# mkangquantum/quits

Hardware: AMD Instinct MI355X
Metric: decoded shots/sec + logical-error-rate, [[144,12,12]] BB code, d rounds, p=0.003 (higher is better)
Workload: dtype f32

## Files before the change

quits_amd/csrc/bp_scatter_wide.hip:

```cpp
#include "qd_internal.h"
#include "qd_host.h"
#include "../../include/quits_amd.h"
#include "bp_scatter_edge.h"

#define QSW_GATHER_PRIO(j_) if ((j_) == 0) __builtin_amdgcn_s_setprio(0); else if ((j_) == CPL - 1) __builtin_amdgcn_s_setprio(2); else __builtin_amdgcn_s_setprio(1);

template <int T, int MW, int CPL, int NSW>
__global__ void __launch_bounds__(T, MW) qd_bp_scatter_wide_kernel(BpGraphDev g, ScatGraphDev sg, DecodeArgs a, ScatArgs x)
{
    extern __shared__ __align__(16) unsigned char smem[];
    const uint32_t lds_base = (uint32_t)(uintptr_t)(__attribute__((address_space(3))) unsigned char *)smem;
    if (lds_base != 0u) __builtin_trap();
    uint32_t *outw = reinterpret_cast<uint32_t *>(smem + sg.off_out);
    int *misc = reinterpret_cast<int *>(smem + sg.off_misc);
    constexpr int NW = T / 64;
    static_assert(T % 64 == 0 && NW <= 16, "workgroup shape");

    const int tid = threadIdx.x;
    const int64_t shot = blockIdx.x;
    const uint8_t *det = a.det + shot * a.det_stride + a.det_offset;
    const uint8_t *upd = a.upd ? a.upd + shot * a.upd_stride : nullptr;
    const int m_pad = g.m_pad, n_pad = g.n_pad;

    int any = 0;
// ... 284 lines not shown
            }
            return;
        }
    }
    for (int b = tid; b < sg.nslots; b += T)
        if (*QS_LDS(cur + 4u * (uint32_t)b) < 0) {
            const uint32_t jf = sg.slot_fault[b];
            if (jf != 0xFFFFFFFFu) atomicOr(&outw[jf >> 5], 1u << (jf & 31u));
        }
    if (!converged && a.want_llr && tid == 0) misc[48] = atomicAdd(a.fail_count, 1);
    __syncthreads();
    for (int w = tid; w < g.out_words; w += T) a.err_bits[shot * g.out_words + w] = outw[w];
    if (!converged && a.want_llr) {
        const int slot = misc[48];
        float *dst = a.llr_ws + (int64_t)slot * n_pad;
        for (int k1 = tid; k1 < g.n; k1 += T) dst[k1] = (float)(*QS_LDS(cur + 4u * sg.k1_slot[k1]) + 1) * x.grid_inv;
        if (tid == 0) a.fail_list[slot] = (int32_t)shot;
    }
    if (tid == 0) a.status[shot] = t | (converged * QD_STATUS_CONVERGED) | a.status_or;
}

#undef QS_ACC
#define QS_ACC(off) (prior_g[((uint32_t)(off) - (uint32_t)sg.offA) >> 2])
#define QS_ADJ(row_) qs_as_uint4(__builtin_amdgcn_raw_buffer_load_b128(adj_rsrc, adj_voff, (row_) * adj_row, 0))
template <int NSW>
__global__ void __launch_bounds__(64) qd_bp_first_pass_kernel(BpGraphDev g, ScatGraphDev sg, const int32_t *prior_g, uint32_t *rec)
{
    static_assert(NSW == 3, "the record has room for three sign words");
    const int c = (int)blockIdx.x * 64 + (int)threadIdx.x;
    const bool actv = c < g.m;
    constexpr int j = 0;
// ... 66 lines not shown
```

quits_amd/csrc/graph_layout.h:

```cpp
#pragma once
#include "qd_graph_views.h"

#include <cstddef>
#include <memory>
#include <type_traits>
#include <utility>
#include <vector>

#define QD_GEN_PREFIX_LDS (32 * 1024)

int qd_fail(int code, const char *fmt, ...);

struct Switches {
    bool no_scatter, scatter_cpl1, scatter_wide_t704, scatter_natural_rounds, scatter_banks_by_slot, scatter_walk_greedy, osdcs_old, bp_no_fast_start;
    float scatter_m2_limit;
    std::vector<int> gen_stages;
};
Switches qd_read_switches();

struct HostGraph {
    int m = 0, n = 0, nnz = 0, max_rdeg = 0, max_cdeg = 0, min_rdeg = 0, m_pad = 0, n_pad = 0, max_rdeg_pad = 0;
    const int32_t *row_ptr = nullptr, *col_idx = nullptr;
    const double *priors = nullptr;
    std::vector<int> rdeg, cdeg;
    std::vector<double> llr0;
    std::vector<int32_t> cp, ri, pos;
    std::vector<int> chk_orig, chk_slot_of, bit_orig, bit_slot_of;
    std::vector<uint8_t> chk_deg;
};
int qd_host_graph(int32_t m, int32_t n, const int32_t *row_ptr, const int32_t *col_idx, const double *priors, HostGraph &h);
// ... 39 lines not shown
```

quits_amd/csrc/graph_layout.hip:

```cpp
#include "graph_layout.h"
#include "../../include/quits_amd.h"

#include <algorithm>
#include <cmath>
#include <cstdlib>
#include <cstring>
#include <numeric>


static inline int align16(int x) { return (x + 15) & ~15; }
static inline int pad64(int x) { return (x + 63) & ~63; }

Switches qd_read_switches()
{
    auto env = [](const char *name) { return std::getenv(name); };
    Switches w{};
    w.no_scatter = env("QD_NO_SCATTER") != nullptr;
    w.scatter_cpl1 = env("QD_SCATTER_CPL1") != nullptr;
    w.scatter_wide_t704 = env("QD_SCATTER_WIDE_T704") != nullptr;
    w.scatter_natural_rounds = env("QD_SCATTER_NATURAL_ROUNDS") != nullptr;
    w.scatter_banks_by_slot = env("QD_SCATTER_BANKS_BY_SLOT") != nullptr;
    w.scatter_walk_greedy = env("QD_SCATTER_WALK_GREEDY") != nullptr;
    const char *ev = env("QD_BP_NO_FAST_START");
    w.bp_no_fast_start = ev && std::atoi(ev) == 1;
    ev = env("QD_OSDCS_OLD");
    w.osdcs_old = ev && std::atoi(ev) == 1;
    ev = env("QD_SCATTER_M2_LIMIT");
    w.scatter_m2_limit = ev ? (float)std::atof(ev) : INFINITY;
    w.gen_stages = {3, 6, 10, 14, 20, 28, 40, 56, 80, 112};
    if ((ev = env("QD_GEN_STAGES"))) {
        w.gen_stages.clear();
        for (const char *q = ev; *q;) {
            char *end = nullptr;
            const long v = std::strtol(q, &end, 10);
            if (end == q) break;
            if (v > 0) w.gen_stages.push_back((int)v);
            q = *end ? end + 1 : end;
        }
    }
    return w;
}

static void scatter_banks(int m, int n, const int32_t *row_ptr, const int32_t *col_idx, const std::vector<int> &chk_orig,
// ... 647 lines not shown
```

quits_amd/csrc/osd_shared.h:

```cpp
#pragma once
#include "qd_internal.h"

#define QD_NOKEY 0xFFFFFFFFu

#ifdef QD_OSD_TIMING
#define QD_TICK(slot)                                                                   \
    {                                                                                   \
        const unsigned long long now_ = wall_clock64();                                 \
        acc_[slot] += now_ - tick_;                                                     \
        tick_ = now_;                                                                   \
    }
#else
#define QD_TICK(slot)
#endif

__device__ __forceinline__ uint64_t &qd_qword(uint64_t *q_lds, uint64_t *q_glb, int kw_lds, int m_pad, int w, int r)
{
    return (w < kw_lds) ? q_lds[(size_t)w * m_pad + r] : q_glb[(size_t)(w - kw_lds) * m_pad + r];
}

__device__ __forceinline__ uint32_t qd_mono_key(float llr)
{
    const float f = llr + 0.0f;
    const uint32_t u = __float_as_uint(f);
    return (u & 0x80000000u) ? ~u : (u | 0x80000000u);
}

template <int T>
__device__ __forceinline__ void qd_bitonic_u64(uint64_t *buf, int P, int tid)
{
    for (int k = 2; k <= P; k <<= 1)
        for (int j = k >> 1; j > 0; j >>= 1) {
            for (int pi = tid; pi < (P >> 1); pi += T) {
                const int i = ((pi & ~(j - 1)) << 1) | (pi & (j - 1));
                const int l = i | j;
                const uint64_t x = buf[i], y = buf[l];
                const bool up = ((i & k) == 0);
                if ((x > y) == up) { buf[i] = y; buf[l] = x; }
            }
            __syncthreads();
// ... 34 lines not shown
    const uint8_t *det, *upd;
    int64_t det_stride, det_offset, upd_stride;
    const float *llr_ws;
    const int32_t *fail_list, *fail_count;
    const int32_t *slot_list, *slot_count;
    uint64_t *q_spill_fast;
    uint64_t *mt_ws;
    uint32_t *err_bits;
    int32_t *status;
    unsigned long long *dbg;
};

struct TierState {
    uint32_t lo_key, lo_idx; int sphase, exhausted, limit;
    uint32_t guess = 0u, cut = 0u, count = 0u;
};

template <int T, int KPT = QD_OSD_KPT, class ARGS = OsdRegArgs, int SCAN = 0>
__device__ __forceinline__ int qd_osd_draw_tier(const ARGS &a, const float *llr, uint64_t *sortbuf, uint16_t *order,
                                             uint32_t *red, uint32_t *sumbuf, TierState &ts)
{
    const int tid = threadIdx.x;
    const int n = a.n;
    const bool in_regs = n <= KPT * T;
    uint32_t lo_key = ts.lo_key, lo_idx = ts.lo_idx;
    int sphase = ts.sphase;
    const uint32_t lim = (uint32_t)ts.limit;
    bool exhausted = false;
    int cnt = 0;
    {
            uint32_t kreg[KPT];
            if (in_regs) {
#pragma unroll
                for (int i = 0; i < KPT; ++i) {
                    const int b = tid + i * T;
                    kreg[i] = (b < n) ? qd_mono_key(llr[b]) : 0xFFFFFFFFu;
                }
            }
            auto scan_keys = [&](auto fn) {
                if constexpr (SCAN == 0) {
                    for (int b = tid; b < n; b += T) fn(qd_mono_key(llr[b]), b);
                } else {
                    const float4 *l4 = reinterpret_cast<const float4 *>(llr);
                    const int n4 = n >> 2;
                    for (int b0 = 0; b0 < n4; b0 += SCAN * T) {
                        float4 v[SCAN > 0 ? SCAN : 1];
#pragma unroll
                        for (int u = 0; u < SCAN; ++u) {
                            const int b4 = b0 + u * T + tid;
                            v[u] = l4[b4 < n4 ? b4 : 0];
                        }
#pragma unroll
                        for (int u = 0; u < SCAN; ++u) {
                            const int b4 = b0 + u * T + tid;
// ... 7 lines not shown
                }
            };
            auto count_ties = [&](uint32_t key, uint32_t ilo, uint32_t ihi) -> uint32_t {
                uint32_t c = 0;
                for (int b = tid; b < n; b += T)
                    if (qd_mono_key(llr[b]) == key) { const uint32_t j = a.bit_orig[b]; c += (j >= ilo && j < ihi) ? 1u : 0u; }
                return qd_block_sum<T>(c, sumbuf, sphase);
            };
            bool by_index = false;
            uint32_t t_lo = lo_key, t_hi = lo_key, i_lo = 0, i_hi = 0;
            if (lo_idx > 0) {
                if (count_ties(lo_key, lo_idx, 0xFFFFFFFFu) > 0) by_index = true;
                else { lo_key += 1; lo_idx = 0; }
            }
            bool spec = !by_index && !in_regs && ts.guess > lo_key;
            for (;;) {
            if (spec) { t_lo = lo_key; t_hi = (uint32_t)__builtin_amdgcn_readfirstlane((int)ts.guess); }
            else {
            if (!by_index) {
                uint32_t *hist = reinterpret_cast<uint32_t *>(sortbuf);
                uint32_t base = 0u, cur_lo = lo_key, cum = 0u;
                uint64_t thi64 = 0;
                for (int level = 0; level < 3; ++level) {
                    const int shift = level == 0 ? 21 : (level == 1 ? 10 : 0);
                    const int nb = level == 2 ? 1024 : 2048;
                    for (int i = tid; i < nb; i += T) hist[i] = 0u;
                    __syncthreads();
                    auto tally = [&](uint32_t u) {
                        if (u != 0xFFFFFFFFu && u >= cur_lo) {
                            const uint32_t bin = (u - base) >> shift;
                            if (bin < (uint32_t)nb) atomicAdd(&hist[bin], 1u);
                        }
// ... 84 lines not shown
            scan_keys([&](uint32_t u, int b) {
                bool take = false;
                uint32_t j = 0;
                if (by_index) { if (u == t_lo) { j = a.bit_orig[b]; take = (j >= i_lo && j < i_hi); } }
                else if (u >= t_lo && u < t_hi) { j = a.bit_orig[b]; take = true; }
                if (take) {
                    const uint32_t at = atomicAdd(&red[80], 1u);
                    if (at < (uint32_t)QD_OSD_TIER) sortbuf[at] = ((uint64_t)u << 32) | j;
                }
            });
            __syncthreads();
            if (!spec) break;
            {
                const uint32_t c = (uint32_t)__builtin_amdgcn_readfirstlane((int)red[80]);
                ts.count = c;
                if (c > 0u && c <= lim) { cnt = (int)c; lo_key = t_hi; ts.cut = t_hi; break; }
                spec = false;
                __syncthreads();
            }
            }
            int P = 64;
            while (P < cnt) P <<= 1;
            for (int i = cnt + tid; i < P; i += T) sortbuf[i] = ~0ull;
            __syncthreads();
            if (cnt <= 256 && cnt <= T) {
                if ((tid & ~63) < cnt) {
                    const uint64_t mine = tid < cnt ? sortbuf[tid] : ~0ull;
                    const uint4 *sb4 = reinterpret_cast<const uint4 *>(sortbuf);
                    int rank = 0;
                    for (int i = 0; i < (cnt + 1) / 2; ++i) {
                        const uint4 v = sb4[i];
                        const uint64_t k0 = (uint64_t)v.x | ((uint64_t)v.y << 32), k1 = (uint64_t)v.z | ((uint64_t)v.w << 32);
                        rank += (k0 < mine ? 1 : 0) + (k1 < mine ? 1 : 0);
                    }
                    if (tid < cnt) order[rank] = (uint16_t)(mine & 0xFFFFu);
                }
            } else {
                qd_bitonic_u64<T>(sortbuf, P, tid);
                for (int i = tid; i < cnt; i += T) order[i] = (uint16_t)(sortbuf[i] & 0xFFFFu);
            }
            __syncthreads();
    }
    ts.lo_key = lo_key; ts.lo_idx = lo_idx; ts.sphase = sphase; ts.exhausted = 0;
    return cnt;
}

struct OsdLds {
    uint64_t *q;
    uint64_t *tb;
    uint8_t *sp;
    int16_t *rowpiv;
    uint16_t *prow;
    uint32_t *pcol;
    uint32_t *pairs;
    uint32_t *bcols;
    uint32_t *red;
    uint32_t *outw;
};
// ... 176 lines not shown
```

quits_amd/csrc/osd_sr.hip:

```cpp
#include "osd_shared.h"
#include "qd_host.h"
#include <algorithm>

#define QD_SR_KWR 4
struct OsdSrArgs {
    int m, n, m_pad, n_pad, mw, out_words, upd_rows, ell_log2;
    int o_tb, o_rowpiv, o_prow, o_pcol, o_ppos, o_nz, o_cand, o_stq, o_stsp, o_bcols, o_red, o_out, o_order;
    int tier_first;
    const uint16_t *csc_ell;
    const uint32_t *bit_orig;
    const uint8_t *det, *upd;
    int64_t det_stride, det_offset, upd_stride;
    const float *llr_ws;
    const int32_t *fail_list, *fail_count;
    uint64_t *q_spill;
    int32_t *hard_list, *hard_count;
    uint32_t *err_bits;
    int32_t *status;
    unsigned long long *dbg;
};

template <int T, int RPT, int KWR>
__global__ void __launch_bounds__(T, qd_sr_wps(RPT)) qd_osd0_sr_kernel(OsdSrArgs a)
{
    extern __shared__ __align__(16) unsigned char smem[];
    const int tid = threadIdx.x, lane = tid & 63;
    constexpr int NW = T / 64;
    static_assert(NW <= 16 && T >= 256, "key / flag records hold 16 wavefronts; the tier drawing wants >= 256 threads");
    uint64_t *tb = reinterpret_cast<uint64_t *>(smem + a.o_tb);
// ... 2 lines not shown
    uint16_t *prow = reinterpret_cast<uint16_t *>(smem + a.o_prow);
    uint32_t *pcol = reinterpret_cast<uint32_t *>(smem + a.o_pcol);
    uint16_t *ppos = reinterpret_cast<uint16_t *>(smem + a.o_ppos);
    uint64_t *nz = reinterpret_cast<uint64_t *>(smem + a.o_nz);
    uint32_t *cand = reinterpret_cast<uint32_t *>(smem + a.o_cand);
    uint64_t *stq = reinterpret_cast<uint64_t *>(smem + a.o_stq);
    uint32_t *stsp = reinterpret_cast<uint32_t *>(smem + a.o_stsp);
    uint32_t *bcols = reinterpret_cast<uint32_t *>(smem + a.o_bcols);
    uint32_t *red = reinterpret_cast<uint32_t *>(smem + a.o_red);
    uint32_t *sumbuf = red + 96;
    uint32_t *outw = reinterpret_cast<uint32_t *>(smem + a.o_out);
    uint16_t *order = reinterpret_cast<uint16_t *>(smem + a.o_order);
    const int m = a.m, m_pad = a.m_pad, mw = a.mw, dlog = a.ell_log2;
    uint64_t *qglb = a.q_spill + (size_t)blockIdx.x * (size_t)(mw > KWR ? mw - KWR : 0) * m_pad;
    const int nfail = *a.fail_count;
    if (tid == 0) red[81] = 0u;
    for (int item = blockIdx.x; item < nfail; item += gridDim.x) {
        const int slot = item;
        const int64_t shot = a.fail_list[slot];
        const float *llr = a.llr_ws + (int64_t)slot * a.n_pad;
        const uint8_t *det = a.det + shot * a.det_stride + a.det_offset;
        const uint8_t *upd = a.upd ? a.upd + shot * a.upd_stride : nullptr;
#ifdef QD_OSD_TIMING
        unsigned long long acc_[12] = {0, 0, 0, 0, 0, 0, 0, 0, 0, 0, 0, 0};
        unsigned long long tick_ = wall_clock64();
#endif
        uint64_t my_tb[RPT], my_q[RPT][KWR];
        uint32_t my_sp = 0, my_piv = 0;
#pragma unroll
        for (int i = 0; i < RPT; ++i) {
// ... 11 lines not shown
        }
        for (int w = tid; w < a.out_words; w += T) outw[w] = 0u;
        if (tid < 240) cand[tid] = (tid % 80) < 64 ? QD_NOKEY : 0u;
        if (tid == 0) red[72] = 0u;
        __syncthreads();
        QD_TICK(10)

        int npiv = 0, done = 0, draining = 0, cmaxp1 = 64, sphase = 0, rd = 0, bseq = 0, ntier = 0;
        uint32_t my_bp = 0;
        uint32_t lo_key = 0, lo_idx = 0;
        while (!done) {
            TierState ts{lo_key, lo_idx, sphase, 0, ntier == 0 ? a.tier_first : QD_OSD_TIER};
            const bool first_tier = ntier == 0;
            if (first_tier) ts.guess = red[81];
            ++ntier;
            const int cnt = qd_osd_draw_tier<T, QD_OSD_KPT, OsdSrArgs, 6>(a, llr, sortbuf, order, red, sumbuf, ts);
            lo_key = ts.lo_key; lo_idx = ts.lo_idx; sphase = ts.sphase;
            if (first_tier) {
                const uint32_t lim1 = (uint32_t)a.tier_first, step = 1u << 20;
                uint32_t g = ts.guess;
                if (ts.cut) g = ts.count * 20u > lim1 * 17u ? ts.cut - step : (ts.count * 20u < lim1 * 11u ? ts.cut + step : ts.cut);
                else if (g) g = ts.count > lim1 ? g - step : g;
                if (g > 0xFFFFFFFFu - step) g = 0u;
                if (tid == 0) red[81] = g;
            }
            QD_TICK(0)
            if (ts.exhausted) break;
            for (int base = 0; base < cnt && !done; base += 64, ++bseq) {
                const int nb = min(64, cnt - base);
#pragma unroll
                for (int i = 0; i < RPT; ++i) { const int r = tid + i * T; if (r < m_pad) tb[r] = 0ull; }
                if (tid < mw) nz[tid] = 0ull;
                if (tid < 64) bcols[tid] = tid < nb ? (uint32_t)order[base + tid] : 0xFFFFFFFFu;
// ... 179 lines not shown
            if (draining && ((my_bp >> i) & 1u) && (int)(ppos[rowpiv[r]] & 63u) >= cmaxp1) ++over;
        }
        const uint32_t tot = qd_block_sum<T>(over | (resid << 16), sumbuf, sphase);
        const int inconsistent = (tot >> 16) != 0u;
        const int npiv_rep = npiv - (int)(tot & 0xFFFFu);
        if (inconsistent) {
            if (tid == 0) a.hard_list[atomicAdd(a.hard_count, 1)] = slot;
        } else {
#pragma unroll
            for (int i = 0; i < RPT; ++i)
                if (((my_piv >> i) & 1u) && ((my_sp >> i) & 1u)) {
                    const uint32_t j = pcol[rowpiv[tid + i * T]];
                    atomicOr(&outw[j >> 5], 1u << (j & 31u));
                }
            __syncthreads();
            for (int w = tid; w < a.out_words; w += T) a.err_bits[shot * a.out_words + w] = outw[w];
            if (tid == 0) a.status[shot] = (a.status[shot] & 0xFFFF) | (1 << 17) | (min(npiv_rep, 4095) << 20);
        }
        QD_TICK(3)
#ifdef QD_OSD_TIMING
        if (tid == 0) {
            for (int i = 0; i < 8; ++i) atomicAdd(&a.dbg[i], acc_[i]);
            atomicAdd(&a.dbg[8], 1ull); atomicAdd(&a.dbg[9], (unsigned long long)npiv); atomicAdd(&a.dbg[10], acc_[10]); atomicAdd(&a.dbg[11], acc_[11]); atomicAdd(&a.dbg[12], (unsigned long long)ntier); atomicAdd(&a.dbg[13], (unsigned long long)bseq);
        }
#endif
        __syncthreads();
    }
}

int qd_osd_sr_layout(int m, int m_pad, int n, int out_words, int *off13, int *threads, int *rpt)
{
    if (m > 2048 || n > 49152) return 0;
    const int T = m <= 256 ? 256 : 512;
    *threads = T; *rpt = (m + T - 1) / T;
    auto al = [](int x) { return (x + 15) & ~15; };
    int o = 0;
    off13[0] = o; o += al(std::max(m_pad * 8, QD_OSD_TIER * 8));
    off13[1] = o; o += al(m_pad * 2);
    off13[2] = o; o += al(m_pad * 2);
    off13[3] = o; o += al(m_pad * 4);
    off13[4] = o; o += al(m_pad * 2);
// ... 3 lines not shown
    off13[8] = o; o += 64 * 4;
    off13[9] = o; o += 64 * 4;
    off13[10] = o; o += 1024;
    off13[11] = o; o += al(out_words * 4);
    off13[12] = o; o += al(QD_OSD_TIER * 2);
    return o;
}

size_t qd_osd_sr_ws_words(int m_pad, int mw, int threads, int rpt)
{
    (void)threads;
    (void)rpt;
    return (size_t)(mw > QD_SR_KWR ? mw - QD_SR_KWR : 0) * m_pad + 64;
}

hipError_t qd_launch_osd0_sr(const OsdGraphDev &g, const BpGraphDev &bg, const DecodeArgs &a, int blocks, hipStream_t s)
{
    OsdSrArgs r{};
    r.m = g.m; r.n = g.n; r.m_pad = g.m_pad; r.n_pad = bg.n_pad; r.mw = g.mw; r.out_words = bg.out_words; r.upd_rows = a.upd_rows;
    r.ell_log2 = g.ell_log2;
    const int *o = g.s_off;
    r.o_tb = o[0]; r.o_rowpiv = o[1]; r.o_prow = o[2]; r.o_pcol = o[3]; r.o_ppos = o[4]; r.o_nz = o[5]; r.o_cand = o[6]; r.o_stq = o[7];
    r.o_stsp = o[8]; r.o_bcols = o[9]; r.o_red = o[10]; r.o_out = o[11]; r.o_order = o[12];
    r.tier_first = QD_OSD_TIER_FIRST;
    r.csc_ell = g.csc_ell; r.bit_orig = bg.bit_orig;
    r.det = a.det; r.upd = a.upd; r.det_stride = a.det_stride; r.det_offset = a.det_offset; r.upd_stride = a.upd_stride;
    r.llr_ws = a.llr_ws; r.fail_list = a.fail_list; r.fail_count = a.fail_count; r.q_spill = a.q_spill_sr;
    r.hard_list = a.hard_list; r.hard_count = a.hard_count;
    r.err_bits = a.err_bits; r.status = a.status; r.dbg = a.dbg;
    const int lds = g.s_lds_bytes;
#define QD_SR_CASE(TT, RR)                                                                                                        \
    {                                                                                                                             \
        auto k = qd_osd0_sr_kernel<TT, RR, QD_SR_KWR>;                                                                     \
        hipError_t e = hipFuncSetAttribute((const void *)k, hipFuncAttributeMaxDynamicSharedMemorySize, lds);                     \
        if (e != hipSuccess) return e;                                                                                            \
        hipLaunchKernelGGL(k, dim3((unsigned)blocks), dim3(TT), lds, s, r);                                                       \
        return hipGetLastError();                                                                                                 \
    }
    if (g.s_threads == 256) {
        switch (g.s_rpt) {
        case 1: QD_SR_CASE(256, 1)
        case 2: QD_SR_CASE(256, 2)
// ... 13 lines not shown
```

quits_amd/csrc/qd_decoder.hip:

```cpp
#include "qd_host.h"

#include <cmath>
#include <cstring>

#define QD_GRID_MIN_BITS 10

extern "C" int qd_decoder_create(const qd_graph *g, const qd_params *p, qd_decoder **out)
{
    if (!g || !p || !out) return qd_fail(QD_EINVAL, "null argument");
    *out = nullptr;
    if (p->bp_method != QD_BP_MINIMUM_SUM && p->bp_method != QD_BP_PRODUCT_SUM) return qd_fail(QD_EINVAL, "unknown bp_method %d", p->bp_method);
    if (p->schedule != QD_SCHEDULE_PARALLEL && p->schedule != QD_SCHEDULE_SERIAL) return qd_fail(QD_EINVAL, "unknown schedule %d", p->schedule);
    if (p->reserved & ~(QD_FLAG_EDGE_MESSAGES | QD_FLAG_RAW_LLR | QD_FLAG_OFF_CHIP)) return qd_fail(QD_EINVAL, "unknown flag bits 0x%x", p->reserved);
    const bool lsd = p->osd_method == QD_LSD_0 || p->osd_method == QD_LSD_E || p->osd_method == QD_LSD_CS;
    if (lsd && p->osd_order < 0) return qd_fail(QD_EINVAL, "negative lsd_order");
    const bool off_chip = g->off_chip || (p->reserved & QD_FLAG_OFF_CHIP);
    if (off_chip && lsd)
        return qd_fail(QD_EUNSUPPORTED, "BP-LSD is not implemented for the off-chip window %d x %d%s", g->m, g->n, g->off_chip ? "" : " (QD_FLAG_OFF_CHIP)");
    if (p->osd_method == QD_LSD_CS && p->osd_order > 64)
        return qd_fail(QD_EUNSUPPORTED, "lsd_cs: lsd_order %d > 64 is not implemented on the device path", p->osd_order);
    if (p->osd_method == QD_LSD_E && p->osd_order > 15)
        return qd_fail(QD_EUNSUPPORTED, "lsd_e: lsd_order %d > 15 is not implemented on the device path", p->osd_order);
    if (lsd && qd_lsd_lds_bytes(g->m, g->n, g->bp.out_words) > QD_LDS_BYTES)
        return qd_fail(QD_ECAPACITY, "window %d x %d does not fit the LSD kernel's LDS layout", g->m, g->n);
// ... 81 lines not shown
                const long long v = std::llround(std::ldexp((double)on_grid(g->h_llr0[j], d->grid_k), d->grid_k));
                pg[g->h_sc_slot[j]] = (int32_t)v - 1;
                mxp = std::max(mxp, std::llabs(v));
            }
            const long long lim = ((1ll << 23) - mxp) / std::max(1, g->max_cdeg) - 1;
            if (mxp < (1ll << 22) && lim > 0) {
                rc |= d->mem.upload(pg, &d->prior_g);
                d->m2_limit = std::min((float)lim, env.scatter_m2_limit);
                d->bp = BP_SCATTER_WIDE;
                if (!env.bp_no_fast_start && rc == 0) {
                    const std::vector<uint32_t> zero((size_t)g->bp.m_pad * 8, 0u);
                    rc |= d->mem.upload(zero, &d->first_pass);
                    if (rc == 0 && (qd_launch_bp_first_pass(d->bp_fine, g->sc, d->prior_g, const_cast<uint32_t *>(d->first_pass), nullptr) != hipSuccess ||
                                    hipStreamSynchronize(nullptr) != hipSuccess))
                        rc = -1;
                }
            }
        }
        if (rc) { d->mem.release(); delete d; return qd_fail(QD_EHIP, "device allocation failed while building the LLR grid"); }
    }
    *out = d;
    return QD_OK;
}

extern "C" int qd_decoder_create_relay(const qd_graph *g, const qd_params *p, const qd_relay_params *r, const float *gammas, qd_decoder **out)
{
    if (!g || !p || !r || !out) return qd_fail(QD_EINVAL, "null argument");
    *out = nullptr;
    if (p->bp_method != QD_BP_MINIMUM_SUM || p->schedule != QD_SCHEDULE_PARALLEL)
        return qd_fail(QD_EINVAL, "Relay-BP is flooding min-sum: bp_method %d / schedule %d are not QD_BP_MINIMUM_SUM / QD_SCHEDULE_PARALLEL", p->bp_method, p->schedule);
// ... 129 lines not shown
        } else if (d->post == QD_POST_OSD0_SR) {
            ws.post_blocks = ncu * g->osd.s_per_cu;
            HIP_TRY(ws.dev.alloc((size_t)ws.post_blocks * qd_osd_sr_ws_words(g->osd.m_pad, g->osd.mw, g->osd.s_threads, g->osd.s_rpt), &ws.q_spill_sr));
        } else if (d->post == QD_POST_OSD_CS_PANEL) {
            ws.post_blocks = ncu * d->cs_per_cu;
            HIP_TRY(ws.dev.alloc((size_t)ws.post_blocks * qd_osdcs_ws_words(d->cs_variant), &ws.cs_ws));
        }
        const int spill_fast = g->osd.mw - (d->osd_w ? g->osd.w_kw : g->osd.f_kw);
        if (g->osd.f_lds_bytes > 0 && spill_fast > 0)
            HIP_TRY(ws.dev.alloc((size_t)d->osd_blocks_fast * spill_fast * g->osd.m_pad, &ws.q_spill_fast));
        if (d->osd_w && g->osd.w_lds_bytes > 0)
            HIP_TRY(ws.dev.alloc((size_t)d->osd_blocks_fast * ((size_t)g->osd.mw * g->osd.m_pad + 64 * 32), &ws.mt_ws));
        HIP_TRY(ws.dev.alloc((size_t)max_batch, &ws.hard_list));
        HIP_TRY(ws.dev.alloc((size_t)max_batch, &ws.hard_list2));
        HIP_TRY(ws.dev.alloc((size_t)max_batch * g->bp.n_pad, &ws.llr_ws));
        HIP_TRY(ws.dev.alloc((size_t)max_batch, &ws.fail_list));
        if (d->osd_blocks > 0)
            HIP_TRY(ws.dev.alloc((size_t)d->osd_blocks * g->n, &ws.order_ws));
        const int spill_planes = g->osd.mw - g->osd.kw_lds;
        if (d->osd_blocks > 0 && spill_planes > 0)
            HIP_TRY(ws.dev.alloc((size_t)d->osd_blocks * spill_planes * g->osd.m_pad, &ws.q_spill));
    }
    if (d->bp == BP_HBM_EDGE) {
        const bool ps = d->prm.bp_method == QD_BP_PRODUCT_SUM, serial = d->prm.schedule == QD_SCHEDULE_SERIAL;
        const int planes = serial ? 2 : (ps ? 3 : 2);
        const bool pre_plane = serial && g->gen.nslots == 0;
        GenStagePlan &sp = d->ws.gsp;
        sp = GenStagePlan{};
        sp.nbounds = d->gen_nbounds;
        std::copy(d->gen_bounds, d->gen_bounds + d->gen_nbounds, sp.bounds);
// ... 83 lines not shown
    if (B == 0) return QD_OK;
    if (det_offset < 0 || det_stride < det_offset + d->g->m) return qd_fail(QD_EINVAL, "detector slice [%lld, %lld) exceeds the row stride %lld", (long long)det_offset, (long long)(det_offset + d->g->m), (long long)det_stride);
    if (d_upd && (upd_rows < 0 || upd_rows > d->g->m || upd_stride < upd_rows)) return qd_fail(QD_EINVAL, "bad syndrome-update shape");
    return QD_OK;
}

static DecodeArgs decode_args(const qd_decoder *d, const uint8_t *d_det, int64_t det_stride, int64_t det_offset, const uint8_t *d_upd,
                              int64_t upd_stride, int32_t upd_rows, uint32_t *d_err_bits, int32_t *d_status)
{
    DecodeArgs a{};
    a.det = d_det; a.det_stride = det_stride; a.det_offset = det_offset;
    a.upd = d_upd; a.upd_stride = upd_stride; a.upd_rows = d_upd ? upd_rows : 0;
    a.max_iter = d->prm.max_iter; a.ms_scale = (float)d->prm.ms_scaling_factor; a.want_llr = d->post != QD_POST_NONE ? 1 : 0;
    a.err_bits = d_err_bits; a.status = d_status;
    a.llr_ws = d->ws.llr_ws; a.fail_list = d->ws.fail_list; a.fail_count = d->ws.fail_count;
    a.order_ws = d->ws.order_ws; a.q_spill = d->ws.q_spill; a.q_spill_fast = d->ws.q_spill_fast; a.q_spill_sr = d->ws.q_spill_sr; a.mt_ws = d->ws.mt_ws;
    a.hard_list = d->ws.hard_list; a.hard_list2 = d->ws.hard_list2; a.hard_count = d->ws.fail_count + 1;
    a.dbg = reinterpret_cast<unsigned long long *>(d->ws.ctr_base) + 2;
    a.osd_w = d->osd_w; a.osd_order = d->prm.osd_order; a.rank = d->g->rank;
    return a;
}

static int launch_bp(qd_decoder *d, const DecodeArgs &a, int64_t B, hipStream_t s)
{
    const qd_graph *g = d->g;
    GenGraphDev gg = g->gen;
    gg.llr0 = d->llr0_q;
    switch (d->bp) {
    case BP_LDS_EDGE: HIP_TRY(qd_launch_bp_ps_lds(gg, g->bp, a, B, s)); break;
    case BP_GATHER_RAW: HIP_TRY(qd_launch_bp(g->bp, a, B, s)); break;
// ... 59 lines not shown
{
    const qd_graph *g = d->g;
    const int blocks = (int)std::min<int64_t>(B, d->ws.post_blocks);
    const int fast = (int)std::min<int64_t>(B, d->osd_blocks_fast), full = (int)std::min<int64_t>(B, d->osd_blocks);
    switch (d->post) {
    case QD_POST_OSD0_OFFCHIP:
        HIP_TRY(qd_launch_osd0_offchip(g->osd, g->bp, a, g->x_off, g->x_off_sort, g->x_off_order, g->x_kw, g->x_threads, g->x_lds, d->ws.q_spill_off, blocks, s));
        break;
    case QD_POST_LSD:
        HIP_TRY(qd_launch_lsd0(g->gen, g->bp, a, d->ws.lsd_ws, d->ws.post_blocks, blocks, d->lsd_w, d->prm.osd_order, g->osd.wfix, s));
        break;
    case QD_POST_OSD_CS_PANEL:
        HIP_TRY(qd_launch_osdcs(g->osd, g->bp, a, d->cs_off, d->cs_variant, d->cs_lds, d->ws.cs_ws, blocks, s));
        break;
    case QD_POST_OSD0_SR:
        HIP_TRY(qd_launch_osd0_sr(g->osd, g->bp, a, blocks, s));
        HIP_TRY(qd_launch_osd0(g->osd, g->bp, a, fast, full, s, true));
        break;
    default:
        HIP_TRY(qd_launch_osd0(g->osd, g->bp, a, fast, full, s));
    }
    return QD_OK;
}

static int decode_impl(qd_decoder *d, const uint8_t *d_det, int64_t det_stride, int64_t det_offset, const uint8_t *d_upd,
                       int64_t upd_stride, int32_t upd_rows, int64_t B, uint32_t *d_err_bits, int32_t *d_status, int stage,
                       void *stream)
{
    if (!d) return qd_fail(QD_EINVAL, "null decoder");
    if (stage < 1 || stage > 3) return qd_fail(QD_EINVAL, "stage must be 1 (BP), 2 (OSD) or 3 (both)");
    if (int rc = check_batch(d, det_stride, det_offset, d_upd, upd_stride, upd_rows, B)) return rc;
    if (B == 0) return QD_OK;
    if (!d_det || !d_err_bits || !d_status) return qd_fail(QD_EINVAL, "null argument");
    HIP_TRY(hipSetDevice(d->g->device));
    if (B > d->cap && stage == 2) return qd_fail(QD_EINVAL, "OSD stage without a preceding BP stage of this batch size");
    if (int rc = B > d->cap ? qd_decoder_reserve(d, B) : QD_OK) return rc;
    hipStream_t s = reinterpret_cast<hipStream_t>(stream);
    const bool post = d->post != QD_POST_NONE;
    if (stage & 1) {
        d->cset ^= 1;
        d->ws.fail_count = d->ws.ctr_base + 64 * d->cset;
        if (!d->set_clean[d->cset]) {
            HIP_TRY(hipMemsetAsync(d->ws.fail_count, 0, 3 * sizeof(int32_t), s));
            HIP_TRY(hipMemsetAsync(d->ws.fail_count + 40, 0, 2 * sizeof(int32_t), s));
        }
        d->set_clean[d->cset] = false;
        d->last_B = B;
    }
    const DecodeArgs a = decode_args(d, d_det, det_stride, det_offset, d_upd, upd_stride, upd_rows, d_err_bits, d_status);
    auto span = [&](int kind) -> int {
        if (!d->profiling) return QD_OK;
        hipEvent_t t0, t1;
        HIP_TRY(hipEventCreate(&t0)); HIP_TRY(hipEventCreate(&t1));
        d->ev.push_back({kind, t0, t1});
        HIP_TRY(hipEventRecord(t0, s));
        return QD_OK;
    };
    if (stage & 1) {
        if (int rc = span(0)) return rc;
        if (int rc = launch_bp(d, a, B, s)) return rc;
        if (d->profiling) HIP_TRY(hipEventRecord(d->ev.back().t1, s));
    }
// ... 49 lines not shown
    return decode_impl(d, d_det, det_stride, det_offset, d_upd, upd_stride, upd_rows, B, d_err_bits, d_status, stage, stream);
}

extern "C" int qd_osd0_batch(qd_decoder *d, const uint8_t *d_det, int64_t det_stride, int64_t det_offset,
                             const uint8_t *d_upd, int64_t upd_stride, int32_t upd_rows, int64_t B, const float *d_llr,
                             uint32_t *d_err_bits, int32_t *d_status, void *stream)
{
    if (!d) return qd_fail(QD_EINVAL, "null decoder");
    if (d->post == QD_POST_NONE) return qd_fail(QD_EINVAL, "decoder was created with osd_method = off");
    if (int rc = check_batch(d, det_stride, det_offset, d_upd, upd_stride, upd_rows, B)) return rc;
    if (B == 0) return QD_OK;
    if (!d_det || !d_llr || !d_err_bits || !d_status) return qd_fail(QD_EINVAL, "null argument");
    HIP_TRY(hipSetDevice(d->g->device));
    if (int rc = B > d->cap ? qd_decoder_reserve(d, B) : QD_OK) return rc;
    hipStream_t s = reinterpret_cast<hipStream_t>(stream);
    const DecodeArgs a = decode_args(d, d_det, det_stride, det_offset, d_upd, upd_stride, upd_rows, d_err_bits, d_status);
    HIP_TRY(hipMemsetAsync(d->ws.fail_count, 0, 3 * sizeof(int32_t), s));
    d->set_clean[d->cset] = false;
    HIP_TRY(qd_launch_stage_llr(d_llr, d->g->n, d->g->bp.n_pad, d->g->bp.bit_orig, B, d->ws.llr_ws, d->ws.fail_list, d->ws.fail_count,
                                d_status, s));
    return launch_post(d, a, B, s);
}

extern "C" int qd_decoder_debug_counters(qd_decoder *d, uint64_t *out16)
{
    if (!d || !out16 || !d->ws.fail_count) return qd_fail(QD_EINVAL, "no workspace yet");
    HIP_TRY(hipSetDevice(d->g->device));
    HIP_TRY(hipDeviceSynchronize());
    HIP_TRY(hipMemcpy(out16, reinterpret_cast<char *>(d->ws.ctr_base) + 16, 16 * sizeof(uint64_t), hipMemcpyDeviceToHost));
    HIP_TRY(hipMemset(reinterpret_cast<char *>(d->ws.ctr_base) + 16, 0, 16 * sizeof(uint64_t)));
// ... 27 lines not shown
```

quits_amd/csrc/qd_host.h:

```cpp
#pragma once
#include "../../include/quits_amd.h"
#include "qd_internal.h"
#include "graph_layout.h"

#include <algorithm>
#include <vector>

#define HIP_TRY(expr)                                                                                    \
    do {                                                                                                 \
        hipError_t e_ = (expr);                                                                          \
        if (e_ != hipSuccess) return qd_fail(QD_EHIP, "%s: %s", #expr, hipGetErrorString(e_));           \
    } while (0)

struct DevAllocs {
    std::vector<void *> ptrs;
    template <class Tp> hipError_t alloc(size_t count, Tp **out) { return alloc_bytes(count * sizeof(Tp), out); }
    template <class Tp> hipError_t alloc_bytes(size_t bytes, Tp **out)
    {
        void *d = nullptr;
        const hipError_t e = hipMalloc(&d, bytes);
        if (e != hipSuccess) return e;
        ptrs.push_back(d);
        *out = static_cast<Tp *>(d);
        return hipSuccess;
// ... 28 lines not shown
};
int qd_host_rank(qd_graph *g);

enum BpPath {
    BP_LDS_EDGE,
    BP_HBM_EDGE,
    BP_SCATTER_WIDE,
    BP_GATHER_GRID,
    BP_GATHER_RAW,
    BP_RELAY,
};

struct Workspace {
    DevAllocs dev;
    float *llr_ws = nullptr;
    float *marg_ws = nullptr;
    int32_t *fail_list = nullptr, *fail_count = nullptr;
    int32_t *ctr_base = nullptr;
    int32_t *host_fail = nullptr;
    hipEvent_t fail_ready = nullptr;
    bool fail_pending = false;
    uint16_t *order_ws = nullptr;
    uint64_t *q_spill = nullptr, *q_spill_fast = nullptr, *mt_ws = nullptr;
    uint64_t *q_spill_sr = nullptr;
    uint64_t *q_spill_off = nullptr;
    int32_t *hard_list = nullptr, *hard_list2 = nullptr;
    int post_blocks = 0;
    uint64_t *cs_ws = nullptr;
    uint64_t *lsd_ws = nullptr;
    GenWs gws{};
// ... 19 lines not shown
    double fail_frac_hint = -1.0;
    int osd_blocks_fast = 0;
    int cs_off[16] = {0}, cs_variant = 0, cs_lds = 0, cs_per_cu = 0;
    int osd_w = 0;
    int lsd_w = 0;
    int64_t gen_ws_limit = 0;
    int gen_bounds[QD_GEN_MAX_STAGES] = {0}, gen_nbounds = 0;
    int grid_k = -1, grid_kc = -1, grid_floor = 0;
    BpGraphDev bp_fine{}, bp_coarse{};
    const float *llr0_q = nullptr;
    const float *llr0_qc = nullptr;
    bool off_chip = false;
    bool edge_cert = false;
    const int32_t *prior_g = nullptr;
    float m2_limit = 0.f;
    const uint32_t *first_pass = nullptr;
    RelayArgs relay{};
    bool relay_marg_device = false;
    int relay_lds_form = 0;
    DevAllocs mem;
    int profiling = 0;
    struct Span { int kind; hipEvent_t t0, t1; };
    std::vector<Span> ev;
    double acc_ms[4] = {0, 0, 0, 0};
};

struct qd_spmat {
    int device = 0;
    SpmatDev d{};
    DevAllocs mem;
// ... 16 lines not shown

hipError_t qd_launch_bp(const BpGraphDev &g, const DecodeArgs &a, int64_t B, hipStream_t s);
hipError_t qd_launch_bp_scatter_wide(const BpGraphDev &g, const ScatGraphDev &sg, const DecodeArgs &a, const ScatArgs &x, int64_t B, hipStream_t s);
hipError_t qd_launch_bp_first_pass(const BpGraphDev &g, const ScatGraphDev &sg, const int32_t *prior_g, uint32_t *rec, hipStream_t s);
hipError_t qd_launch_bp_general(const GenGraphDev &g, const BpGraphDev &bg, const DecodeArgs &a, const GenWs &w, int bp_method,
                                int schedule, int64_t shot0, int nshots, hipStream_t s, GenStagePlan *plan);
hipError_t qd_launch_bp_relay(const BpGraphDev &g, const DecodeArgs &a, const RelayArgs &x, int64_t B, hipStream_t s);
hipError_t qd_launch_bp_relay_device(const BpGraphDev &g, const DecodeArgs &a, const RelayArgs &x, int64_t B, hipStream_t s);
int qd_relay_layout(const BpGraphDev &g, bool marg_device, RelayArgs *x);
hipError_t qd_launch_hold(const int32_t *count, int threshold, int microseconds, hipStream_t s);
int qd_bp_ps_lds_bytes(const GenGraphDev &g, int max_rdeg);
hipError_t qd_launch_bp_ps_lds(const GenGraphDev &g, const BpGraphDev &bg, const DecodeArgs &a, int64_t B, hipStream_t s);
hipError_t qd_launch_osd0(const OsdGraphDev &g, const BpGraphDev &bg, const DecodeArgs &a, int blocks_fast,
                          int blocks_full, hipStream_t s, bool handed_over = false);
int qd_osd_sr_layout(int m, int m_pad, int n, int out_words, int *off13, int *threads, int *rpt);
hipError_t qd_launch_osd0_sr(const OsdGraphDev &g, const BpGraphDev &bg, const DecodeArgs &a, int blocks, hipStream_t s);
int qd_osdcs_layout(int m, int n, int out_words, uint32_t max_wfix, int *off, int *variant, int *per_cu);
size_t qd_osdcs_ws_words(int variant);
hipError_t qd_launch_osdcs(const OsdGraphDev &g, const BpGraphDev &bg, const DecodeArgs &a, const int *off, int variant, int lds,
                           uint64_t *ws, int blocks, hipStream_t s);
size_t qd_osd_sr_ws_words(int m_pad, int mw, int threads, int rpt);
int qd_osd_offchip_layout(int m, int n, int max_cdeg, int *off, int *off_sort, int *off_order, int *kw, int *threads, int *per_cu);
size_t qd_osd_offchip_ws_words(int m, int kw);
hipError_t qd_launch_osd0_offchip(const OsdGraphDev &g, const BpGraphDev &bg, const DecodeArgs &a, const int *off, int off_sort, int off_order,
                                  int kw, int threads, int lds, uint64_t *q_ws, int blocks, hipStream_t s);
hipError_t qd_launch_lsd0(const GenGraphDev &gg, const BpGraphDev &bg, const DecodeArgs &d, uint64_t *q_ws, int blocks_alloc, int blocks,
                          int lsd_w, int lsd_order, const uint32_t *wfix, hipStream_t s);
size_t qd_lsd_ws_bytes(int m, int n, int blocks, int lsd_w);
int qd_lsd_lds_bytes(int m, int n, int out_words);
hipError_t qd_launch_stage_llr(const float *llr_in, int n, int n_pad, const uint32_t *bit_orig, int64_t B, float *llr_ws,
                               int32_t *fail_list, int32_t *fail_count, int32_t *status, hipStream_t s);
// ... 28 lines not shown
```

quits_amd/csrc/qd_internal.h:

```cpp
#pragma once
#include <hip/hip_runtime.h>
#include <stdint.h>
#include "qd_graph_views.h"

#define QD_WAVE 64

struct ScatArgs {
    const int32_t *prior_g;
    float grid_inv;
    float m2_limit;
    int32_t *recheck_list;
    int32_t *recheck_count;
    int recheck_cap;
    const uint32_t *first_pass;
};

struct GenWs {
    float *b2c, *c2b, *th, *llr;
    float *pre;
    uint8_t *syn;
    int32_t *slot;
    int64_t S;
};
static inline bool qd_event_done(hipEvent_t e)
// ... 150 lines not shown
```

Before: 1.650 million.

## Emit low-LLR candidate lists from BP for OSD tier selection

When BP fails to converge, the scatter kernel now also writes a per-shot list of bits whose monotone LLR key falls below an adaptive cut, into a new candidate workspace. The OSD-SR first tier reads this list instead of scanning and histogramming all n LLRs, and gains a rank sort for 257-512 candidates. The cut is adjusted between calls from overflow and underflow counts. This adds global atomics and writes to the BP failure path, more workspace memory, and a feedback heuristic that may miss or over-collect candidates.

```diff
diff --git a/quits_amd/csrc/bp_scatter_wide.hip b/quits_amd/csrc/bp_scatter_wide.hip
--- a/quits_amd/csrc/bp_scatter_wide.hip
+++ b/quits_amd/csrc/bp_scatter_wide.hip
@@ -322,7 +322,22 @@
     if (!converged && a.want_llr) {
         const int slot = misc[48];
         float *dst = a.llr_ws + (int64_t)slot * n_pad;
-        for (int k1 = tid; k1 < g.n; k1 += T) dst[k1] = (float)(*QS_LDS(cur + 4u * sg.k1_slot[k1]) + 1) * x.grid_inv;
+        uint64_t *const cws = *reinterpret_cast<uint64_t *const *>(a.fail_count + QD_CTR_CAND);
+        const uint32_t cut = cws ? *reinterpret_cast<const uint32_t *>(cws) : 0u;
+        uint64_t *row = cws + 2 + (int64_t)slot * QD_CAND_ROW, *cl = row + 2;
+        for (int k1 = tid; k1 < g.n; k1 += T) {
+            const float v = (float)(*QS_LDS(cur + 4u * sg.k1_slot[k1]) + 1) * x.grid_inv;
+            dst[k1] = v;
+            const uint32_t key = qd_mono_key(v);
+            if (key < cut) {
+                const uint32_t at = atomicAdd(reinterpret_cast<uint32_t *>(&misc[49]), 1u);
+                if (at < (uint32_t)QD_CAND_CAP) cl[at] = ((uint64_t)key << 32) | (uint32_t)k1;
+            }
+        }
+        if (cut) {
+            __syncthreads();
+            if (tid == 0) *reinterpret_cast<uint4 *>(row) = make_uint4((uint32_t)misc[49], cut, (uint32_t)a.want_llr, (uint32_t)shot);
+        }
         if (tid == 0) a.fail_list[slot] = (int32_t)shot;
     }
     if (tid == 0) a.status[shot] = t | (converged * QD_STATUS_CONVERGED) | a.status_or;
diff --git a/quits_amd/csrc/graph_layout.h b/quits_amd/csrc/graph_layout.h
--- a/quits_amd/csrc/graph_layout.h
+++ b/quits_amd/csrc/graph_layout.h
@@ -14,6 +14,8 @@
 struct Switches {
     bool no_scatter, scatter_cpl1, scatter_wide_t704, scatter_natural_rounds, scatter_banks_by_slot, scatter_walk_greedy, osdcs_old, bp_no_fast_start;
     float scatter_m2_limit;
+    bool osd_no_cand, osd_cand_fixed;
+    float osd_cand_cut;
     std::vector<int> gen_stages;
 };
 Switches qd_read_switches();
diff --git a/quits_amd/csrc/graph_layout.hip b/quits_amd/csrc/graph_layout.hip
--- a/quits_amd/csrc/graph_layout.hip
+++ b/quits_amd/csrc/graph_layout.hip
@@ -27,6 +27,11 @@
     w.osdcs_old = ev && std::atoi(ev) == 1;
     ev = env("QD_SCATTER_M2_LIMIT");
     w.scatter_m2_limit = ev ? (float)std::atof(ev) : INFINITY;
+    ev = env("QD_OSD_NO_CAND");
+    w.osd_no_cand = ev && std::atoi(ev) == 1;
+    ev = env("QD_OSD_CAND_CUT");
+    w.osd_cand_fixed = ev != nullptr;
+    w.osd_cand_cut = ev ? (float)std::atof(ev) : 0.f;
     w.gen_stages = {3, 6, 10, 14, 20, 28, 40, 56, 80, 112};
     if ((ev = env("QD_GEN_STAGES"))) {
         w.gen_stages.clear();
diff --git a/quits_amd/csrc/osd_shared.h b/quits_amd/csrc/osd_shared.h
--- a/quits_amd/csrc/osd_shared.h
+++ b/quits_amd/csrc/osd_shared.h
@@ -17,13 +17,6 @@
 __device__ __forceinline__ uint64_t &qd_qword(uint64_t *q_lds, uint64_t *q_glb, int kw_lds, int m_pad, int w, int r)
 {
     return (w < kw_lds) ? q_lds[(size_t)w * m_pad + r] : q_glb[(size_t)(w - kw_lds) * m_pad + r];
-}
-
-__device__ __forceinline__ uint32_t qd_mono_key(float llr)
-{
-    const float f = llr + 0.0f;
-    const uint32_t u = __float_as_uint(f);
-    return (u & 0x80000000u) ? ~u : (u | 0x80000000u);
 }
 
 template <int T>
@@ -88,11 +81,13 @@
 struct TierState {
     uint32_t lo_key, lo_idx; int sphase, exhausted, limit;
     uint32_t guess = 0u, cut = 0u, count = 0u;
+    uint32_t listed = 0u;
 };
 
-template <int T, int KPT = QD_OSD_KPT, class ARGS = OsdRegArgs, int SCAN = 0>
+template <int T, int KPT = QD_OSD_KPT, class ARGS = OsdRegArgs, int SCAN = 0, bool LIST = false>
 __device__ __forceinline__ int qd_osd_draw_tier(const ARGS &a, const float *llr, uint64_t *sortbuf, uint16_t *order,
-                                             uint32_t *red, uint32_t *sumbuf, TierState &ts)
+                                             uint32_t *red, uint32_t *sumbuf, TierState &ts,
+                                             const uint64_t *cand = nullptr, uint32_t cand_n = 0u, uint32_t cand_cut = 0u)
 {
     const int tid = threadIdx.x;
     const int n = a.n;
@@ -102,6 +97,7 @@
     const uint32_t lim = (uint32_t)ts.limit;
     bool exhausted = false;
     int cnt = 0;
+    [[maybe_unused]] bool use_list = false;
     {
             uint32_t kreg[KPT];
             if (in_regs) {
@@ -112,6 +108,14 @@
                 }
             }
             auto scan_keys = [&](auto fn) {
+                if constexpr (LIST) {
+                    if (use_list) {
+                        uint32_t i = (uint32_t)tid;
+                        asm volatile("" : "+v"(i));
+                        for (; i < cand_n; i += (uint32_t)T) { const uint64_t e = cand[i]; fn((uint32_t)(e >> 32), (int)(uint32_t)e); }
+                        return;
+                    }
+                }
                 if constexpr (SCAN == 0) {
                     for (int b = tid; b < n; b += T) fn(qd_mono_key(llr[b]), b);
                 } else {
@@ -149,8 +153,15 @@
                 else { lo_key += 1; lo_idx = 0; }
             }
             bool spec = !by_index && !in_regs && ts.guess > lo_key;
+            if constexpr (LIST) {
+                use_list = __builtin_amdgcn_readfirstlane((int)(!in_regs && cand_n > 0u && lo_key == 0u && lo_idx == 0u)) != 0;
+                if (use_list) spec = true;
+            }
             for (;;) {
-            if (spec) { t_lo = lo_key; t_hi = (uint32_t)__builtin_amdgcn_readfirstlane((int)ts.guess); }
+            if (spec) {
+                t_lo = lo_key; t_hi = (uint32_t)__builtin_amdgcn_readfirstlane((int)ts.guess);
+                if constexpr (LIST) { if (use_list) t_hi = cand_cut; }
+            }
             else {
             if (!by_index) {
                 uint32_t *hist = reinterpret_cast<uint32_t *>(sortbuf);
@@ -265,7 +276,7 @@
             {
                 const uint32_t c = (uint32_t)__builtin_amdgcn_readfirstlane((int)red[80]);
                 ts.count = c;
-                if (c > 0u && c <= lim) { cnt = (int)c; lo_key = t_hi; ts.cut = t_hi; break; }
+                if (c > 0u && (c <= lim || use_list)) { cnt = (int)c; lo_key = t_hi; ts.cut = t_hi; break; }
                 spec = false;
                 __syncthreads();
             }
@@ -274,7 +285,28 @@
             while (P < cnt) P <<= 1;
             for (int i = cnt + tid; i < P; i += T) sortbuf[i] = ~0ull;
             __syncthreads();
-            if (cnt <= 256 && cnt <= T) {
+            bool by_rank = cnt <= 256 && cnt <= T;
+            if constexpr (LIST) {
+                if (cnt > 256 && cnt <= 512) {
+                    by_rank = false;
+                    const uint4 *sb4 = reinterpret_cast<const uint4 *>(sortbuf);
+                    for (int e = tid; (e & ~63) < cnt; e += T) {
+                        const uint64_t mine = e < cnt ? sortbuf[e] : ~0ull;
+                        int rank = 0;
+                        for (int i = 0; i < (cnt + 1) / 2; ++i) {
+                            const uint4 v = sb4[i];
+                            const uint64_t k0 = (uint64_t)v.x | ((uint64_t)v.y << 32), k1 = (uint64_t)v.z | ((uint64_t)v.w << 32);
+                            rank += (k0 < mine ? 1 : 0) + (k1 < mine ? 1 : 0);
+                        }
+                        if (e < cnt) order[rank] = (uint16_t)(mine & 0xFFFFu);
+                    }
+                    __syncthreads();
+                    ts.lo_key = lo_key; ts.lo_idx = lo_idx; ts.sphase = sphase; ts.exhausted = 0;
+                    ts.listed = use_list ? 1u : 0u;
+                    return cnt;
+                }
+            }
+            if (by_rank) {
                 if ((tid & ~63) < cnt) {
                     const uint64_t mine = tid < cnt ? sortbuf[tid] : ~0ull;
                     const uint4 *sb4 = reinterpret_cast<const uint4 *>(sortbuf);
@@ -293,6 +325,7 @@
             __syncthreads();
     }
     ts.lo_key = lo_key; ts.lo_idx = lo_idx; ts.sphase = sphase; ts.exhausted = 0;
+    if constexpr (LIST) ts.listed = use_list ? 1u : 0u;
     return cnt;
 }
 
diff --git a/quits_amd/csrc/osd_sr.hip b/quits_amd/csrc/osd_sr.hip
--- a/quits_amd/csrc/osd_sr.hip
+++ b/quits_amd/csrc/osd_sr.hip
@@ -13,6 +13,8 @@
     int64_t det_stride, det_offset, upd_stride;
     const float *llr_ws;
     const int32_t *fail_list, *fail_count;
+    uint64_t *cand_ws;
+    uint32_t cand_call, cand_fixed;
     uint64_t *q_spill;
     int32_t *hard_list, *hard_count;
     uint32_t *err_bits;
@@ -45,6 +47,7 @@
     const int m = a.m, m_pad = a.m_pad, mw = a.mw, dlog = a.ell_log2;
     uint64_t *qglb = a.q_spill + (size_t)blockIdx.x * (size_t)(mw > KWR ? mw - KWR : 0) * m_pad;
     const int nfail = *a.fail_count;
+    if (tid == 0) { red[82] = 0u; red[83] = 0u; red[84] = 0u; red[85] = 0u; }
     if (tid == 0) red[81] = 0u;
     for (int item = blockIdx.x; item < nfail; item += gridDim.x) {
         const int slot = item;
@@ -86,9 +89,19 @@
             const bool first_tier = ntier == 0;
             if (first_tier) ts.guess = red[81];
             ++ntier;
-            const int cnt = qd_osd_draw_tier<T, QD_OSD_KPT, OsdSrArgs, 6>(a, llr, sortbuf, order, red, sumbuf, ts);
+            uint32_t cand_n = 0u, cand_cut = 0u;
+            const uint64_t *crow = a.cand_ws + 2 + (int64_t)slot * QD_CAND_ROW;
+            if (a.cand_call) {
+                const uint4 hd = *reinterpret_cast<const uint4 *>(crow);
+                const bool mine = hd.z == a.cand_call && hd.w == (uint32_t)shot && hd.y != 0u;
+                cand_n = (uint32_t)__builtin_amdgcn_readfirstlane((int)((mine && hd.x <= (uint32_t)QD_CAND_CAP) ? hd.x : 0u));
+                cand_cut = (uint32_t)__builtin_amdgcn_readfirstlane((int)hd.y);
+                if (first_tier && tid == 0 && mine && hd.x > (uint32_t)QD_CAND_CAP) red[84] += 1u;
+            }
+            const int cnt = qd_osd_draw_tier<T, QD_OSD_KPT, OsdSrArgs, 6, true>(a, llr, sortbuf, order, red, sumbuf, ts, crow + 2, cand_n, cand_cut);
             lo_key = ts.lo_key; lo_idx = ts.lo_idx; sphase = ts.sphase;
-            if (first_tier) {
+            if (tid == 0 && cand_n) { if (ts.listed) red[85] += 1u; else red[83] += 1u; }
+            if (first_tier && !ts.listed) {
                 const uint32_t lim1 = (uint32_t)a.tier_first, step = 1u << 20;
                 uint32_t g = ts.guess;
                 if (ts.cut) g = ts.count * 20u > lim1 * 17u ? ts.cut - step : (ts.count * 20u < lim1 * 11u ? ts.cut + step : ts.cut);
@@ -298,9 +311,11 @@
                     atomicOr(&outw[j >> 5], 1u << (j & 31u));
                 }
             __syncthreads();
+#pragma unroll 1
             for (int w = tid; w < a.out_words; w += T) a.err_bits[shot * a.out_words + w] = outw[w];
             if (tid == 0) a.status[shot] = (a.status[shot] & 0xFFFF) | (1 << 17) | (min(npiv_rep, 4095) << 20);
         }
+        if (tid == 0) red[82] += 1u;
         QD_TICK(3)
 #ifdef QD_OSD_TIMING
         if (tid == 0) {
@@ -309,6 +324,19 @@
         }
 #endif
         __syncthreads();
+    }
+    if (tid == 0 && a.cand_call && red[82] > 0u) {
+        atomicAdd(&a.dbg[14], (unsigned long long)(red[83] + red[84]));
+        atomicAdd(&a.dbg[15], (unsigned long long)red[85]);
+    }
+    if (blockIdx.x == 0 && tid == 0 && a.cand_call && !a.cand_fixed && red[82] > 0u) {
+        uint32_t *cutw = reinterpret_cast<uint32_t *>(a.cand_ws);
+        const uint32_t cut = *cutw;
+        const auto llr_of = [](uint32_t key) { return __uint_as_float((key & 0x80000000u) ? (key & 0x7FFFFFFFu) : ~key); };
+        float c = 0.f;
+        if (cut == 0u) c = red[81] ? llr_of(red[81]) : 0.f;
+        else c = llr_of(cut) + fminf(2.f, fmaxf(-2.f, 16.f * ((float)red[83] - (float)red[84]) / (float)red[82]));
+        if (cut != 0u || red[81]) *cutw = qd_mono_key(fminf(fmaxf(c, 0.5f), 1.0e30f));
     }
 }
 
@@ -342,7 +370,8 @@
     return (size_t)(mw > QD_SR_KWR ? mw - QD_SR_KWR : 0) * m_pad + 64;
 }
 
-hipError_t qd_launch_osd0_sr(const OsdGraphDev &g, const BpGraphDev &bg, const DecodeArgs &a, int blocks, hipStream_t s)
+hipError_t qd_launch_osd0_sr(const OsdGraphDev &g, const BpGraphDev &bg, const DecodeArgs &a, int blocks, hipStream_t s, uint64_t *cand_ws, uint32_t cand_call,
+                             bool cand_fixed)
 {
     OsdSrArgs r{};
     r.m = g.m; r.n = g.n; r.m_pad = g.m_pad; r.n_pad = bg.n_pad; r.mw = g.mw; r.out_words = bg.out_words; r.upd_rows = a.upd_rows;
@@ -354,6 +383,7 @@
     r.csc_ell = g.csc_ell; r.bit_orig = bg.bit_orig;
     r.det = a.det; r.upd = a.upd; r.det_stride = a.det_stride; r.det_offset = a.det_offset; r.upd_stride = a.upd_stride;
     r.llr_ws = a.llr_ws; r.fail_list = a.fail_list; r.fail_count = a.fail_count; r.q_spill = a.q_spill_sr;
+    r.cand_ws = cand_ws; r.cand_call = cand_ws ? cand_call : 0u; r.cand_fixed = cand_fixed ? 1u : 0u;
     r.hard_list = a.hard_list; r.hard_count = a.hard_count;
     r.err_bits = a.err_bits; r.status = a.status; r.dbg = a.dbg;
     const int lds = g.s_lds_bytes;
diff --git a/quits_amd/csrc/qd_decoder.hip b/quits_amd/csrc/qd_decoder.hip
--- a/quits_amd/csrc/qd_decoder.hip
+++ b/quits_amd/csrc/qd_decoder.hip
@@ -119,6 +119,16 @@
                     if (rc == 0 && (qd_launch_bp_first_pass(d->bp_fine, g->sc, d->prior_g, const_cast<uint32_t *>(d->first_pass), nullptr) != hipSuccess ||
                                     hipStreamSynchronize(nullptr) != hipSuccess))
                         rc = -1;
+                }
+                if (d->post == QD_POST_OSD0_SR && !env.osd_no_cand && g->n > g->osd.s_threads && rc == 0) {
+                    uint32_t key = 0u;
+                    if (env.osd_cand_fixed) {
+                        const float f = env.osd_cand_cut + 0.0f;
+                        uint32_t u;
+                        std::memcpy(&u, &f, 4);
+                        key = (u & 0x80000000u) ? ~u : (u | 0x80000000u);
+                    }
+                    d->cand_lists = true; d->cand_cut0 = key; d->cand_fixed = env.osd_cand_fixed;
                 }
             }
         }
@@ -278,6 +288,14 @@
         HIP_TRY(ws.dev.alloc((size_t)max_batch, &ws.hard_list));
         HIP_TRY(ws.dev.alloc((size_t)max_batch, &ws.hard_list2));
         HIP_TRY(ws.dev.alloc((size_t)max_batch * g->bp.n_pad, &ws.llr_ws));
+        if (d->cand_lists) {
+            const size_t words = 2 + (size_t)max_batch * QD_CAND_ROW;
+            HIP_TRY(ws.dev.alloc(words, &ws.cand_ws));
+            HIP_TRY(hipMemset(ws.cand_ws, 0, words * sizeof(uint64_t)));
+            HIP_TRY(hipMemcpy(ws.cand_ws, &d->cand_cut0, sizeof(uint32_t), hipMemcpyHostToDevice));
+            for (int cs = 0; cs < 2; ++cs)
+                HIP_TRY(hipMemcpy(ws.ctr_base + 64 * cs + QD_CTR_CAND, &ws.cand_ws, sizeof(uint64_t *), hipMemcpyHostToDevice));
+        }
         HIP_TRY(ws.dev.alloc((size_t)max_batch, &ws.fail_list));
         if (d->osd_blocks > 0)
             HIP_TRY(ws.dev.alloc((size_t)d->osd_blocks * g->n, &ws.order_ws));
@@ -391,6 +409,7 @@
     a.max_iter = d->prm.max_iter; a.ms_scale = (float)d->prm.ms_scaling_factor; a.want_llr = d->post != QD_POST_NONE ? 1 : 0;
     a.err_bits = d_err_bits; a.status = d_status;
     a.llr_ws = d->ws.llr_ws; a.fail_list = d->ws.fail_list; a.fail_count = d->ws.fail_count;
+    if (d->ws.cand_ws) a.want_llr = (int)d->cand_call;
     a.order_ws = d->ws.order_ws; a.q_spill = d->ws.q_spill; a.q_spill_fast = d->ws.q_spill_fast; a.q_spill_sr = d->ws.q_spill_sr; a.mt_ws = d->ws.mt_ws;
     a.hard_list = d->ws.hard_list; a.hard_list2 = d->ws.hard_list2; a.hard_count = d->ws.fail_count + 1;
     a.dbg = reinterpret_cast<unsigned long long *>(d->ws.ctr_base) + 2;
@@ -480,7 +499,7 @@
         HIP_TRY(qd_launch_osdcs(g->osd, g->bp, a, d->cs_off, d->cs_variant, d->cs_lds, d->ws.cs_ws, blocks, s));
         break;
     case QD_POST_OSD0_SR:
-        HIP_TRY(qd_launch_osd0_sr(g->osd, g->bp, a, blocks, s));
+        HIP_TRY(qd_launch_osd0_sr(g->osd, g->bp, a, blocks, s, d->ws.cand_ws, d->ws.cand_ws ? (uint32_t)a.want_llr : 0u, d->cand_fixed));
         HIP_TRY(qd_launch_osd0(g->osd, g->bp, a, fast, full, s, true));
         break;
     default:
@@ -509,9 +528,11 @@
         if (!d->set_clean[d->cset]) {
             HIP_TRY(hipMemsetAsync(d->ws.fail_count, 0, 3 * sizeof(int32_t), s));
             HIP_TRY(hipMemsetAsync(d->ws.fail_count + 40, 0, 2 * sizeof(int32_t), s));
+            static_assert(QD_CTR_CAND >= 42 && QD_CTR_CAND + 2 <= 64 && QD_CTR_CAND % 2 == 0, "the fills of a counter set (words 0..2, 40..41; 4..35 are the debug counters) must not reach the list array's address");
         }
         d->set_clean[d->cset] = false;
         d->last_B = B;
+        if (++d->cand_call == 0u) d->cand_call = 1u;
     }
     const DecodeArgs a = decode_args(d, d_det, det_stride, det_offset, d_upd, upd_stride, upd_rows, d_err_bits, d_status);
     auto span = [&](int kind) -> int {
@@ -591,6 +612,7 @@
     HIP_TRY(hipSetDevice(d->g->device));
     if (int rc = B > d->cap ? qd_decoder_reserve(d, B) : QD_OK) return rc;
     hipStream_t s = reinterpret_cast<hipStream_t>(stream);
+    if (++d->cand_call == 0u) d->cand_call = 1u;
     const DecodeArgs a = decode_args(d, d_det, det_stride, det_offset, d_upd, upd_stride, upd_rows, d_err_bits, d_status);
     HIP_TRY(hipMemsetAsync(d->ws.fail_count, 0, 3 * sizeof(int32_t), s));
     d->set_clean[d->cset] = false;
diff --git a/quits_amd/csrc/qd_host.h b/quits_amd/csrc/qd_host.h
--- a/quits_amd/csrc/qd_host.h
+++ b/quits_amd/csrc/qd_host.h
@@ -66,6 +66,7 @@
 struct Workspace {
     DevAllocs dev;
     float *llr_ws = nullptr;
+    uint64_t *cand_ws = nullptr;
     float *marg_ws = nullptr;
     int32_t *fail_list = nullptr, *fail_count = nullptr;
     int32_t *ctr_base = nullptr;
@@ -115,6 +116,10 @@
     bool edge_cert = false;
     const int32_t *prior_g = nullptr;
     float m2_limit = 0.f;
+    bool cand_lists = false;
+    uint32_t cand_cut0 = 0;
+    bool cand_fixed = false;
+    uint32_t cand_call = 0;
     const uint32_t *first_pass = nullptr;
     RelayArgs relay{};
     bool relay_marg_device = false;
@@ -161,7 +166,8 @@
 hipError_t qd_launch_osd0(const OsdGraphDev &g, const BpGraphDev &bg, const DecodeArgs &a, int blocks_fast,
                           int blocks_full, hipStream_t s, bool handed_over = false);
 int qd_osd_sr_layout(int m, int m_pad, int n, int out_words, int *off13, int *threads, int *rpt);
-hipError_t qd_launch_osd0_sr(const OsdGraphDev &g, const BpGraphDev &bg, const DecodeArgs &a, int blocks, hipStream_t s);
+hipError_t qd_launch_osd0_sr(const OsdGraphDev &g, const BpGraphDev &bg, const DecodeArgs &a, int blocks, hipStream_t s, uint64_t *cand_ws = nullptr,
+                             uint32_t cand_call = 0, bool cand_fixed = false);
 int qd_osdcs_layout(int m, int n, int out_words, uint32_t max_wfix, int *off, int *variant, int *per_cu);
 size_t qd_osdcs_ws_words(int variant);
 hipError_t qd_launch_osdcs(const OsdGraphDev &g, const BpGraphDev &bg, const DecodeArgs &a, const int *off, int variant, int lds,
diff --git a/quits_amd/csrc/qd_internal.h b/quits_amd/csrc/qd_internal.h
--- a/quits_amd/csrc/qd_internal.h
+++ b/quits_amd/csrc/qd_internal.h
@@ -4,6 +4,17 @@
 #include "qd_graph_views.h"
 
 #define QD_WAVE 64
+#define QD_CAND_CAP 1024
+#define QD_CAND_ROW (QD_CAND_CAP + 2)
+#define QD_CTR_CAND 48
+
+__device__ __forceinline__ uint32_t qd_mono_key(float llr)
+{
+    const float f = llr + 0.0f;
+    const uint32_t u = __float_as_uint(f);
+    return (u & 0x80000000u) ? ~u : (u | 0x80000000u);
+}
+
 
 struct ScatArgs {
     const int32_t *prior_g;
```

Measured after the change: 1.663 million, median of 6. About the same (+0.8%).
